# hazenai/SqueezeDet-PyTorch

Measured on AMD Instinct MI355X. Metric: images/sec SqueezeDet 1248x384 bs=20 inference (+ training under "train"), higher is better.
Workload: dtype f32; 1 GPU; SqueezeDet KITTI 1248x384 bs=20 inference on 1 MI355X (Fire+ConvDet HIP kernels, fused NMS); arch=squeezedet, global_batch=20, input=3x384x1248 fp32 NCHW, HBM resident, weights=synthetic Kaiming-scale, seed 1234, parallelism=replicas x1, steps_in_flight=2

## Files before the change

squeezedet-pytorch_amd/csrc/conv_wino.hip:

```cpp
#include "sqd_common.h"
#include "wino_tile.h"
#include <type_traits>

struct WinoArgs {
  const float* x; const float* u; const float* bias; float* y;
  int B, H, W;
  int C, x_pitch, x_coff;
  int N, Npad, y_pitch, y_coff;
  int relu, accumulate;
  const float* ymask; const float* ymul;
  int gxn, gyn;
  unsigned gxn_m, gyn_m;
  int ngroups, ntiles;
  int nslices, gx;
  int wg_cap;
  int nslices3, N1, y_coff1;
  const float* bias1;
  const float* br_w; const float* br_bias; const float* br_sqb;
  int br_nsq;
  int pb_hp, pb_wp, pb_ns, pb_nseg, pb_gseg, pb_ng;
  float* sv; int sv_pitch, sv_coff, sv_coff1;
  unsigned char* sv_codes;
};

typedef __attribute__((address_space(3))) void* lds_ptr_w_t;

template <int NT, int WV>
__global__ __launch_bounds__(WV * 64, (WV == 4 && NT == 2) ? 2 : ((WV == 4 && NT == 1) ? 3 : 1)) void conv_wino_kernel(WinoArgs a) {
#if defined(__HIP_DEVICE_COMPILE__)
  constexpr int NTHR = WV * 64;
  constexpr int BN = 16 * NT;
  constexpr int RAW_IT = 4;
  constexpr int USLOTS = 32 * BN;
  static_assert(USLOTS % NTHR == 0, "U slice must be whole workgroup passes");
  constexpr int U_IT = USLOTS / NTHR;
  constexpr int NDMA = RAW_IT + U_IT;
  constexpr int NSTEP = 8;
  extern __shared__ __attribute__((aligned(16))) float smem[];
  float* const rawB = smem;
  float* const VB = rawB + WV * 256 * 4;
  float* const UB = VB + WV * 1024 * NT;

  const int tid = threadIdx.x, lane = tid & 63, wv = tid >> 6;
  const int lr = lane & 15, g = lane >> 4;
  const int wgq = (int)blockIdx.x >> 3;
  const int n0 = (wgq % a.nslices) * BN;
  const int tstride = a.gx;
  const int nchunks = a.C >> 3;
  const int ntiles = a.ntiles;
  int tile = ((int)blockIdx.x & 7) * (a.gx >> 3) + wgq / a.nslices;
  if (tile >= ntiles) return;
  const int wv_s = __builtin_amdgcn_readfirstlane(wv);

  int r_offB[RAW_IT], r_key[RAW_IT];
#pragma unroll
  for (int it = 0; it < RAW_IT; ++it) wino_patch_slot(it * 64 + lane, a.W, a.x_pitch, r_offB[it], r_key[it]);
  int u_offB[U_IT];
#pragma unroll
  for (int it = 0; it < U_IT; ++it) {
    const int slot = it * NTHR + tid;
    const int pp = slot / (4 * BN), rem = slot - pp * (4 * BN);
    u_offB[it] = ((pp * a.Npad + n0) * 16 + rem * 4) * 4;
  }
  const unsigned u_chunkB = 16u * a.Npad * 8u * 4u;
  const __amdgpu_buffer_rsrc_t xres = __builtin_amdgcn_make_buffer_rsrc(
      (void*)(a.x + a.x_coff - (long long)(a.W + 1) * a.x_pitch), 0, 0x7ffffff0, 0x00020000);
  const __amdgpu_buffer_rsrc_t ures = __builtin_amdgcn_make_buffer_rsrc((void*)a.u, 0, 0x7ffffff0, 0x00020000);

  typedef WinoGPos GPos;
  auto group_pos = [&](int t) { return wino_group_pos(a, t * WV + wv_s); };
  int r_offG[RAW_IT];
  auto group_offsets = [&](const GPos gp) { wino_group_offsets<RAW_IT>(gp.y0, gp.x0, gp.inner, a.H, a.W, r_offB, r_key, r_offG); };
  float* const rawW = rawB + wv_s * 256 * 4;
  float* const VW = VB + wv_s * 1024 * NT;
  auto dma_raw_one = [&](int it, unsigned soff) {
    __builtin_amdgcn_raw_ptr_buffer_load_lds(xres, (lds_ptr_w_t)(rawW + it * 64 * 4), 16, r_offG[it], (int)soff, 0, 0);
  };
  auto dma_u_one = [&](int it, int cc, int buf) {
    __builtin_amdgcn_raw_ptr_buffer_load_lds(ures, (lds_ptr_w_t)(UB + (buf * USLOTS + it * NTHR + wv_s * 64) * 4), 16, u_offB[it],
                                             (int)(cc * u_chunkB), 0, 0);
  };

  f32x4 acc[16][NT];
#pragma unroll
  for (int p = 0; p < 16; ++p)
#pragma unroll
    for (int j = 0; j < NT; ++j) acc[p][j] = (f32x4){0.f, 0.f, 0.f, 0.f};

  f32x4 biasv[NT];
#pragma unroll
  for (int j = 0; j < NT; ++j) {
    const int n = n0 + j * 16 + 4 * g;
    biasv[j] = (a.bias && n < a.N) ? *(const f32x4*)(a.bias + n) : (f32x4){0.f, 0.f, 0.f, 0.f};
  }
  const int ty = lr >> 3, tx = lr & 7;
  int o_off[4];
#pragma unroll
  for (int px = 0; px < 4; ++px) o_off[px] = ((2 * ty + (px >> 1)) * a.W + 2 * tx + (px & 1)) * a.y_pitch + 4 * g;
  const float relu_lo = a.relu ? 0.f : -__builtin_inff();

  const float* const rawL = rawW + (((g >> 1) * WINO_RP + (2 * (lr >> 3)) * 18 + 2 * (lr & 7)) * 4 + 2 * (g & 1));
  const float* const uR0 = UB + g * 64 + lr * 4;
  f32x4* const parkW = (f32x4*)VW + lane;

  GPos cur = group_pos(tile);
  group_offsets(cur);
#pragma unroll
  for (int it = 0; it < RAW_IT; ++it) dma_raw_one(it, cur.soff);
#pragma unroll
  for (int it = 0; it < U_IT; ++it) dma_u_one(it, 0, 0);
  int ubuf = 0;
  bool pending = false;
  GPos ptp = cur;

  const int acc_i = a.accumulate, has_mul = a.ymul != nullptr, has_mask = a.ymask != nullptr;
  auto epi = [&](f32x4 v, int j, float* dst, const float* mul, const float* mask) {
    if (acc_i) v += *(const f32x4*)dst;
    if (has_mul) v *= *(const f32x4*)mul;
    if (has_mask) {
      const f32x4 m = *(const f32x4*)mask;
      v.x = m.x > 0.f ? v.x : 0.f; v.y = m.y > 0.f ? v.y : 0.f; v.z = m.z > 0.f ? v.z : 0.f; v.w = m.w > 0.f ? v.w : 0.f;
    }
    *(f32x4*)dst = wino_relu4(v, relu_lo);
  };
  auto flush = [&](const GPos gp) {
    float* ybase = a.y + gp.p0 * a.y_pitch + a.y_coff + n0;
    const float* mulbase = a.ymul + gp.p0 * a.y_pitch + a.y_coff + n0;
    const float* maskbase = a.ymask + gp.p0 * a.y_pitch + a.y_coff + n0;
    const bool whole = gp.y0 + 4 <= a.H && gp.x0 + 16 <= a.W && n0 + BN <= a.N;
    if (!gp.valid) return;
    if (whole) {
#pragma unroll
      for (int px = 0; px < 4; ++px)
#pragma unroll
        for (int j = 0; j < NT; ++j) {
          const int off = o_off[px] + j * 16;
          epi(parkW[(px * NT + j) * 64], j, ybase + off, mulbase + off, maskbase + off);
        }
      return;
    }
#pragma unroll
    for (int px = 0; px < 4; ++px) {
      const bool valid = gp.y0 + 2 * ty + (px >> 1) < a.H && gp.x0 + 2 * tx + (px & 1) < a.W;
#pragma unroll
      for (int j = 0; j < NT; ++j) {
        if (!valid || n0 + j * 16 + 4 * g >= a.N) continue;
        const int off = o_off[px] + j * 16;
        epi(parkW[(px * NT + j) * 64], j, ybase + off, mulbase + off, maskbase + off);
      }
    }
  };

  for (;;) {
    const int more_i = (int)((unsigned)(tile + tstride - ntiles) >> 31);
    const bool more = more_i != 0;
    const GPos nxt = group_pos(more ? tile + tstride : tile);
    for (int cc = 0; cc < nchunks; ++cc) {
      asm volatile("s_waitcnt vmcnt(0)" ::: "memory");
      __syncthreads();
      if (pending) { flush(ptp); pending = false; }
      const int last_i = 1 - (int)((unsigned)(cc + 1 - nchunks) >> 31);
      const bool last = last_i != 0;
      const int ncc = last ? 0 : cc + 1;
      if (last) group_offsets(nxt);
      const unsigned nsoff = (last ? nxt.soff : cur.soff) + (unsigned)ncc * 32u;

      f32x2 vv[16];
      wino_input_transform(rawL, vv);
      asm volatile("s_waitcnt lgkmcnt(0)" ::: "memory");
      __builtin_amdgcn_sched_barrier(0);
      const float* const uR = uR0 + ubuf * USLOTS * 4;

      auto load_ops = [&](int step, f32x4 (&afr)[NT]) {
#pragma unroll
        for (int j = 0; j < NT; ++j) afr[j] = *(const f32x4*)(uR + (step * NT + j) * 256);
      };
      auto mfma_phase = [&](auto first_c) {
      constexpr bool FIRST = decltype(first_c)::value;
      auto mfma_pos = [&](int step, const f32x4 (&afr)[NT], int h) {
        const int p = 2 * step + h;
#pragma unroll
        for (int t = 0; t < 2; ++t)
#pragma unroll
          for (int j = 0; j < NT; ++j) {
            const f32x4 c0v = (FIRST && t == 0) ? ((p == 5) ? biasv[j] : (f32x4){0.f, 0.f, 0.f, 0.f}) : acc[p][j];
            acc[p][j] = mfma16(afr[j][2 * h + t], vv[p][t], c0v);
          }
      };
      f32x4 af0[NT], af1[NT];
      load_ops(0, af0);
#pragma unroll
      for (int step = 0; step < NSTEP; ++step) {
#pragma unroll
        for (int q = 0; q < NDMA; ++q) {
          if (q * NSTEP / NDMA != step) continue;
          if (q < RAW_IT) dma_raw_one(q < RAW_IT ? q : 0, nsoff);
          else dma_u_one(q - RAW_IT, ncc, ubuf ^ 1);
        }
        if (step & 1) {
          mfma_pos(step, af1, 0);
          __builtin_amdgcn_sched_barrier(0);
          if (step + 1 < NSTEP) load_ops(step + 1, af0);
          __builtin_amdgcn_sched_barrier(0);
          mfma_pos(step, af1, 1);
        } else {
          mfma_pos(step, af0, 0);
          __builtin_amdgcn_sched_barrier(0);
          if (step + 1 < NSTEP) load_ops(step + 1, af1);
          __builtin_amdgcn_sched_barrier(0);
          mfma_pos(step, af0, 1);
        }
      }
      };
      if (cc == 0) mfma_phase(std::true_type{}); else mfma_phase(std::false_type{});

      if (last) {
#pragma unroll
        for (int j = 0; j < NT; ++j) {
          f32x4 ov[4];
          wino_inverse(acc, j, ov);
#pragma unroll
          for (int px = 0; px < 4; ++px) parkW[(px * NT + j) * 64] = ov[px];
        }
        pending = true; ptp = cur;
      }
      ubuf ^= 1;
    }
    if (!more) break;
    tile += tstride;
    cur = nxt;
  }
  if (pending) flush(ptp);
  asm volatile("s_waitcnt vmcnt(0)" ::: "memory");
#endif
}

template <int NT, int WV, bool USTAT, bool E1>
__device__ __forceinline__ void wino_pipe_body(const WinoArgs& a) {
  static_assert(USTAT, "streamed-U form retired");
  static_assert(!E1 || NT == 2, "expand1x1 slices are built on the 32-channel tiling");
  constexpr int NTHR = WV * 64;
  constexpr int BN = 16 * NT;
  constexpr int RAW_IT = 4;
  constexpr int USLOTS = 32 * BN;
  static_assert(USLOTS % NTHR == 0, "U slice must be whole workgroup passes");
  constexpr int U_IT = USLOTS / NTHR;
  constexpr int NDMA = RAW_IT;
  constexpr int NST = 4 * NT;
  constexpr int NSTEP = 8;
  constexpr int RAW_STEPS = 4;
  extern __shared__ __attribute__((aligned(16))) float smem[];
  float* const rawB = smem;
  float* const UB = rawB + 2 * WV * 256 * 4;

  const int tid = threadIdx.x, lane = tid & 63, wv = tid >> 6;
  const int lr = lane & 15, g = lane >> 4;
  const int wgq = (int)blockIdx.x >> 3;
  const int n0 = (wgq % a.nslices) * BN;
  const int tstride = a.gx;
  const int nchunks = a.C >> 3;
  const int ntiles = a.ntiles;
  int tile = ((int)blockIdx.x & 7) * (a.gx >> 3) + wgq / a.nslices;
  if (tile >= ntiles) return;
  const int wv_s = __builtin_amdgcn_readfirstlane(wv);

  int r_offB[RAW_IT], r_key[RAW_IT];
#pragma unroll
  for (int it = 0; it < RAW_IT; ++it) wino_patch_slot(it * 64 + lane, a.W, a.x_pitch, r_offB[it], r_key[it]);
  int u_offB[U_IT];
#pragma unroll
  for (int it = 0; it < U_IT; ++it) {
    const int slot = it * NTHR + tid;
    const int pp = slot / (4 * BN), rem = slot - pp * (4 * BN);
    u_offB[it] = ((pp * a.Npad + n0) * 16 + rem * 4) * 4;
  }
  const unsigned u_chunkB = 16u * a.Npad * 8u * 4u;
  const __amdgpu_buffer_rsrc_t xres = __builtin_amdgcn_make_buffer_rsrc(
      (void*)(a.x + a.x_coff - (long long)(a.W + 1) * a.x_pitch), 0, 0x7ffffff0, 0x00020000);
  const __amdgpu_buffer_rsrc_t ures = __builtin_amdgcn_make_buffer_rsrc((void*)a.u, 0, 0x7ffffff0, 0x00020000);

  typedef WinoGPos GPos;
  auto group_pos = [&](int t) { return wino_group_pos(a, t * WV + wv_s); };
  int r_offG[RAW_IT];
  auto group_offsets = [&](int y0, int x0, int inner) { wino_group_offsets<RAW_IT>(y0, x0, inner, a.H, a.W, r_offB, r_key, r_offG); };
  float* const rawW = rawB + wv_s * 256 * 4;
  auto dma_raw_one = [&](int it, unsigned soff, int rb) {
    __builtin_amdgcn_raw_ptr_buffer_load_lds(xres, (lds_ptr_w_t)(rawW + (rb * WV * 256 + it * 64) * 4), 16, r_offG[it], (int)soff, 0, 0);
  };
  auto dma_u_one = [&](int it, int cc, int slot) {
    __builtin_amdgcn_raw_ptr_buffer_load_lds(ures, (lds_ptr_w_t)(UB + (slot * USLOTS + it * NTHR + wv_s * 64) * 4), 16, u_offB[it],
                                             (int)(cc * u_chunkB), 0, 0);
  };

  f32x4 acc[16][NT];
#pragma unroll
  for (int p = 0; p < 16; ++p)
#pragma unroll
    for (int j = 0; j < NT; ++j) acc[p][j] = (f32x4){0.f, 0.f, 0.f, 0.f};
  f32x4 biasv[NT];
#pragma unroll
  for (int j = 0; j < NT; ++j) {
    const int n = n0 + j * 16 + 4 * g;
    biasv[j] = (!E1 && a.bias && n < a.N) ? *(const f32x4*)(a.bias + n) : (f32x4){0.f, 0.f, 0.f, 0.f};
  }
  const int e1_c0 = E1 ? (n0 - a.nslices3 * BN) * 4 : 0;
  float e1_biasA[E1 ? 8 : 1];
  const float e1_oneB = (g == 0) ? 1.f : 0.f;
  if constexpr (E1) {
#pragma unroll
    for (int blk = 0; blk < 8; ++blk) {
      const int ch = e1_c0 + blk * 16 + lr;
      e1_biasA[blk] = (g == 0 && a.bias1 && ch < a.N1) ? a.bias1[ch] : 0.f;
    }
  }
  const int ty = lr >> 3, tx = lr & 7;
  int o_offB[4];
#pragma unroll
  for (int px = 0; px < 4; ++px) o_offB[px] = (((2 * ty + (px >> 1)) * a.W + 2 * tx + (px & 1)) * a.y_pitch + 4 * g) * 4;
  const __amdgpu_buffer_rsrc_t yres = __builtin_amdgcn_make_buffer_rsrc((void*)(E1 ? a.y + a.y_coff1 + e1_c0 : a.y + a.y_coff + n0), 0, 0x7ffffff0, 0x00020000);
  const __amdgpu_buffer_rsrc_t mulres = __builtin_amdgcn_make_buffer_rsrc((void*)(a.ymul ? a.ymul + a.y_coff + n0 : a.y), 0, 0x7ffffff0, 0x00020000);
  const __amdgpu_buffer_rsrc_t maskres = __builtin_amdgcn_make_buffer_rsrc((void*)(a.ymask ? a.ymask + a.y_coff + n0 : a.y), 0, 0x7ffffff0, 0x00020000);
  const float relu_lo = a.relu ? 0.f : -__builtin_inff();
  const int rawL_off = (((g >> 1) * WINO_RP + (2 * (lr >> 3)) * 18 + 2 * (lr & 7)) * 4 + 2 * (g & 1));
// ... 500 lines not shown
```

squeezedet-pytorch_amd/csrc/wino_poolbridge.h:

```cpp
template <int NSQ, int NCH, bool SAVE = false>
__device__ __forceinline__ void wino_poolbridge16_body(const WinoArgs& a) {
  constexpr int WV = 8, NTHR = WV * 64, RAW_IT = 4, RSLOTS = 224;
  extern __shared__ __attribute__((aligned(16))) float smem[];
  const int P3 = a.nslices3, P = a.nslices;
  constexpr int nchunks = NCH;
  const bool e1_half = a.N1 <= 64;
  const int e1_stage = e1_half ? 1024 : 2048;
  const int rb1 = e1_half ? 2 : 4;
  float* const rawB = smem;
  float* const UB = rawB + 2 * WV * RSLOTS * 4;
  float* const U1B = UB + P3 * nchunks * 2048;
  float* const sqAL = U1B + (P - P3) * nchunks * e1_stage;
  const int nblk = P3 + rb1 * (P - P3);
  float* const biasL = sqAL + nblk * 4 * NSQ * 64;
  float* const sqbL = biasL + P * 64;

  const int tid = threadIdx.x, lane = tid & 63, wv = tid >> 6;
  const int lr = lane & 15, g = lane >> 4;
  const int ntasks = a.ngroups;
  const int wv_s = __builtin_amdgcn_readfirstlane(wv);
  int task = (int)blockIdx.x * WV + wv_s;
  const int tstride = a.gx * WV;

  int r_offB[RAW_IT], r_key[RAW_IT];
#pragma unroll
  for (int it = 0; it < RAW_IT; ++it) wino_patch_slot(it * 64 + lane, a.W, a.x_pitch, r_offB[it], r_key[it]);
  const __amdgpu_buffer_rsrc_t xres = __builtin_amdgcn_make_buffer_rsrc(
      (void*)(a.x + a.x_coff - (long long)(a.W + 1) * a.x_pitch), 0, 0x7ffffff0, 0x00020000);
  const __amdgpu_buffer_rsrc_t ures = __builtin_amdgcn_make_buffer_rsrc((void*)a.u, 0, 0x7ffffff0, 0x00020000);
  const __amdgpu_buffer_rsrc_t yres = __builtin_amdgcn_make_buffer_rsrc(
      (void*)(a.y + a.y_coff - (long long)a.pb_wp * a.y_pitch), 0, 0x7ffffff0, 0x00020000);
  const __amdgpu_buffer_rsrc_t pres = __builtin_amdgcn_make_buffer_rsrc(
      (void*)((SAVE ? a.sv : a.y) - (SAVE ? (long long)a.pb_wp * a.sv_pitch : 0)), 0, 0x7ffffff0, 0x00020000);
  const __amdgpu_buffer_rsrc_t cres = __builtin_amdgcn_make_buffer_rsrc(
      (void*)(SAVE ? (void*)(a.sv_codes - (long long)a.pb_wp * a.sv_pitch) : (void*)a.y), 0, 0x7ffffff0, 0x00020000);

  {
    const int u_lane = (g * 16 + lr) * 16;
    const unsigned u_chunkB = 16u * a.Npad * 8u * 4u;
    for (int ps = 0; ps < P; ++ps)
      for (int c = 0; c < nchunks; ++c) {
        const bool is1 = ps >= P3;
        if (is1 && e1_half && (wv_s & 1)) continue;
        float* const dst = is1 ? U1B + ((ps - P3) * nchunks + c) * e1_stage + (e1_half ? (wv_s >> 1) : wv_s) * 256
                               : UB + (ps * nchunks + c) * 2048 + wv_s * 256;
        __builtin_amdgcn_raw_ptr_buffer_load_lds(ures, (lds_ptr_w_t)dst, 16, u_lane + wv_s * a.Npad * 64,
                                                 (int)(c * u_chunkB + (unsigned)ps * 1024u), 0, 0);
      }
    for (int i = tid; i < nblk * 4 * NSQ * 64; i += NTHR) sqAL[i] = a.br_w[i];
    for (int i = tid; i < P * 64; i += NTHR) biasL[i] = a.br_bias[i];
    for (int i = tid; i < NSQ * 16; i += NTHR) sqbL[i] = (a.br_sqb && i < a.br_nsq) ? a.br_sqb[i] : 0.f;
  }
  asm volatile("s_waitcnt vmcnt(0)" ::: "memory");
  __syncthreads();
  if (task >= ntasks) return;

  struct IterPos { int b, s, r, y0, x0, inner; unsigned soff; };
  auto iter_pos = [&](int b, int s, int r) {
    IterPos ip;
    ip.b = b; ip.s = s; ip.r = r;
    ip.y0 = 4 * r; ip.x0 = 14 * s;
    const long long p0 = ((long long)b * a.H + ip.y0) * a.W + ip.x0;
    ip.soff = (unsigned)(p0 * a.x_pitch * 4);
    ip.inner = (int)(((unsigned)(-ip.y0) & (unsigned)(ip.y0 + 4 - a.H) & (unsigned)(-ip.x0) & (unsigned)(ip.x0 + 16 - a.W)) >> 31);
    return ip;
  };
  float* const rawW = rawB + wv_s * RSLOTS * 4;
  auto dma_group = [&](const IterPos& ip) {
#pragma unroll
    for (int it = 0; it < RAW_IT; ++it) {
      const int key = r_key[it];
      const bool ok = ip.inner ? true : (key >= 0 && (unsigned)(ip.y0 + (key >> 8) - 1) < (unsigned)a.H && (unsigned)(ip.x0 + (key & 255) - 1) < (unsigned)a.W);
      const int off = ok ? r_offB[it] : (int)WINO_OOB;
      if (it < RAW_IT - 1 || lane < RSLOTS - (RAW_IT - 1) * 64) {
        __builtin_amdgcn_raw_ptr_buffer_load_lds(xres, (lds_ptr_w_t)(rawW + (it * 64) * 4), 16, off, (int)ip.soff, 0, 0);
        if (nchunks > 1)
          __builtin_amdgcn_raw_ptr_buffer_load_lds(xres, (lds_ptr_w_t)(rawW + (WV * RSLOTS + it * 64) * 4), 16, off, (int)(ip.soff + 32u), 0, 0);
      }
    }
  };
  auto task_of = [&](int q, int& b, int& s, int& g0, int& g1) {
    const int v = q % a.pb_nseg; const int q1 = q / a.pb_nseg;
    s = q1 % a.pb_ns; b = q1 / a.pb_ns;
    g0 = v * a.pb_gseg; g1 = g0 + a.pb_gseg < a.pb_ng ? g0 + a.pb_gseg : a.pb_ng;
  };

  f32x4 acc[16];
  f32x4 acc_sq[NSQ];
  f32x4 carry[8];
  unsigned carry_code[SAVE ? 8 : 1];
#pragma unroll
  for (int k = 0; k < 8; ++k) carry[k] = (f32x4){0.f, 0.f, 0.f, 0.f};
#pragma unroll
  for (int k = 0; k < (SAVE ? 8 : 1); ++k) carry_code[k] = 0u;
  const float oneB = (g == 0) ? 1.f : 0.f;
  const int ty = lr >> 3, tx = lr & 7;
  const int o_off = (((1 - ty) * a.pb_wp + tx) * a.y_pitch + 4 * g) * 4;
  const int p_off = SAVE ? (((1 - ty) * a.pb_wp + tx) * a.sv_pitch + 4 * g) * 4 : 0;
  const int rawL_off = (((g >> 1) * WINO_RP + (2 * (lr >> 3)) * 18 + 2 * (lr & 7)) * 4 + 2 * (g & 1));
  const int u_ln = g * 64 + lr * 4;
  auto max4 = [](f32x4 p, f32x4 q) {
    f32x4 r;
    r.x = __builtin_fmaxf(p.x, q.x); r.y = __builtin_fmaxf(p.y, q.y); r.z = __builtin_fmaxf(p.z, q.z); r.w = __builtin_fmaxf(p.w, q.w);
    return r;
  };
  auto shl = [](float v, auto n_c) {
    constexpr int N = decltype(n_c)::value;
    return __builtin_bit_cast(float, __builtin_amdgcn_update_dpp(0, __builtin_bit_cast(int, v), 0x100 + N, 0xf, 0xf, true));
  };
  auto shr = [](float v, auto n_c) {
    constexpr int N = decltype(n_c)::value;
    return __builtin_bit_cast(float, __builtin_amdgcn_update_dpp(0, __builtin_bit_cast(int, v), 0x110 + N, 0xf, 0xf, true));
  };

  int tb, ts, g0, g1;
  task_of(task, tb, ts, g0, g1);
  int r = g0;
  IterPos cur = iter_pos(tb, ts, r);
  dma_group(cur);
  bool stored = false;

  for (;;) {
    const int rlast = (g1 < a.pb_ng || 2 * a.pb_ng - 1 < a.pb_hp) ? g1 : g1 - 1;
    int nb = tb, ns = ts, ng0 = g0, ng1 = g1, nr = r + 1, ntask = task;
    bool more = true;
    if (r >= rlast) {
      ntask = task + tstride;
      more = ntask < ntasks;
      if (more) { task_of(ntask, nb, ns, ng0, ng1); nr = ng0; } else { nr = r; }
    }
    if (stored && (!SAVE || nblk == 8)) asm volatile("s_waitcnt vmcnt(%0)" ::"n"(NSQ + (SAVE ? 16 : 0)) : "memory");
    else asm volatile("s_waitcnt vmcnt(0)" ::: "memory");
    asm volatile("" ::: "memory");
    f32x2 vv[NCH][16];
#pragma unroll
    for (int c = 0; c < NCH; ++c) wino_input_transform(rawW + c * WV * RSLOTS * 4 + rawL_off, vv[c]);
    asm volatile("s_waitcnt lgkmcnt(0)" ::: "memory");
    __builtin_amdgcn_sched_barrier(0);
    const IterPos nxt = iter_pos(nb, ns, nr);
    dma_group(nxt);

#pragma unroll
    for (int q = 0; q < NSQ; ++q) acc_sq[q] = (f32x4){0.f, 0.f, 0.f, 0.f};
    const bool wholexy = cur.y0 + 4 <= a.H && cur.x0 + 16 <= a.W;
    const bool emit_px = tx < 7 && 7 * ts + tx < a.pb_wp && 2 * r - ty < a.pb_hp && (ty ? (r > g0) : (r < g1));
    const unsigned psoff = SAVE ? (unsigned)((((long long)tb * a.pb_hp + 2 * r) * a.pb_wp + 7 * ts) * a.sv_pitch * 4) : 0u;
    auto pool_in = [&](int bi, auto kslot_c, f32x4 (&ov)[4], int cbase, int climit) {
      constexpr int KS = decltype(kslot_c)::value;
      if (!wholexy) {
#pragma unroll
        for (int px = 0; px < 4; ++px)
          if (!(cur.y0 + 2 * ty + (px >> 1) < a.H && cur.x0 + 2 * tx + (px & 1) < a.W)) ov[px] = (f32x4){0.f, 0.f, 0.f, 0.f};
      }
      const f32x4 m_top = max4(ov[0], ov[1]), m_left = max4(ov[0], ov[2]);
      const f32x4 m_all = max4(m_top, max4(ov[2], ov[3]));
      f32x4 A, Bt, pooled;
      const f32x4 ov0 = ov[0];
      asm volatile("s_nop 1\n\t"
                   "v_max_f32_dpp %0, %8, %12 row_shl:1 row_mask:0xf bank_mask:0xf bound_ctrl:1\n\t"
                   "v_max_f32_dpp %1, %9, %13 row_shl:1 row_mask:0xf bank_mask:0xf bound_ctrl:1\n\t"
                   "v_max_f32_dpp %2, %10, %14 row_shl:1 row_mask:0xf bank_mask:0xf bound_ctrl:1\n\t"
                   "v_max_f32_dpp %3, %11, %15 row_shl:1 row_mask:0xf bank_mask:0xf bound_ctrl:1\n\t"
                   "v_max_f32_dpp %4, %16, %20 row_shl:1 row_mask:0xf bank_mask:0xf bound_ctrl:1\n\t"
                   "v_max_f32_dpp %5, %17, %21 row_shl:1 row_mask:0xf bank_mask:0xf bound_ctrl:1\n\t"
                   "v_max_f32_dpp %6, %18, %22 row_shl:1 row_mask:0xf bank_mask:0xf bound_ctrl:1\n\t"
                   "v_max_f32_dpp %7, %19, %23 row_shl:1 row_mask:0xf bank_mask:0xf bound_ctrl:1"
                   : "=&v"(A.x), "=&v"(A.y), "=&v"(A.z), "=&v"(A.w), "=&v"(Bt.x), "=&v"(Bt.y), "=&v"(Bt.z), "=&v"(Bt.w)
                   : "v"(m_left.x), "v"(m_left.y), "v"(m_left.z), "v"(m_left.w), "v"(m_all.x), "v"(m_all.y), "v"(m_all.z), "v"(m_all.w),
                     "v"(ov0.x), "v"(ov0.y), "v"(ov0.z), "v"(ov0.w), "v"(m_top.x), "v"(m_top.y), "v"(m_top.z), "v"(m_top.w));
      f32x4 base;
#pragma unroll
      for (int e = 0; e < 4; ++e) base[e] = ty ? carry[KS][e] : A[e];
      asm volatile("s_nop 1\n\t"
                   "v_max_f32_dpp %0, %4, %8 row_shl:8 row_mask:0xf bank_mask:0xf bound_ctrl:1\n\t"
                   "v_max_f32_dpp %1, %5, %9 row_shl:8 row_mask:0xf bank_mask:0xf bound_ctrl:1\n\t"
                   "v_max_f32_dpp %2, %6, %10 row_shl:8 row_mask:0xf bank_mask:0xf bound_ctrl:1\n\t"
                   "v_max_f32_dpp %3, %7, %11 row_shl:8 row_mask:0xf bank_mask:0xf bound_ctrl:1\n\t"
                   "v_max_f32_dpp %0, %4, %0 row_shr:8 row_mask:0xf bank_mask:0xf bound_ctrl:1\n\t"
                   "v_max_f32_dpp %1, %5, %1 row_shr:8 row_mask:0xf bank_mask:0xf bound_ctrl:1\n\t"
                   "v_max_f32_dpp %2, %6, %2 row_shr:8 row_mask:0xf bank_mask:0xf bound_ctrl:1\n\t"
                   "v_max_f32_dpp %3, %7, %3 row_shr:8 row_mask:0xf bank_mask:0xf bound_ctrl:1"
                   : "=&v"(pooled.x), "=&v"(pooled.y), "=&v"(pooled.z), "=&v"(pooled.w)
                   : "v"(Bt.x), "v"(Bt.y), "v"(Bt.z), "v"(Bt.w), "v"(base.x), "v"(base.y), "v"(base.z), "v"(base.w));
      if constexpr (SAVE) {
        unsigned codes = 0u, cApack = 0u;
#pragma unroll
        for (int e = 0; e < 4; ++e) {
          const float o0 = ov[0][e], o1 = ov[1][e], o2 = ov[2][e], o3 = ov[3][e];
          float r0;
          asm volatile("s_nop 1\n\tv_mov_b32_dpp %0, %1 row_shl:1 row_mask:0xf bank_mask:0xf bound_ctrl:1" : "=&v"(r0) : "v"(o0));
          const float Av = A[e], Bv = Bt[e];
          unsigned cA = 5u;
          cA = (o3 == Av) ? 4u : cA; cA = (o2 == Av) ? 3u : cA; cA = (r0 == Av) ? 2u : cA; cA = (o1 == Av) ? 1u : cA; cA = (o0 == Av) ? 0u : cA;
          const unsigned cB = (o0 == Bv) ? 6u : ((o1 == Bv) ? 7u : 8u);
          unsigned cBn;
          asm volatile("s_nop 1\n\t"
                       "v_mov_b32_dpp %0, %1 row_shl:8 row_mask:0xf bank_mask:0x3 bound_ctrl:1\n\t"
                       "v_mov_b32_dpp %0, %1 row_shr:8 row_mask:0xf bank_mask:0xc bound_ctrl:1" : "=&v"(cBn) : "v"(cB));
          const unsigned cbase_e = ty ? ((carry_code[KS] >> (8 * e)) & 0xffu) : cA;
          unsigned code = (base[e] == pooled[e]) ? cbase_e : cBn;
          code = pooled[e] > 0.f ? code : 15u;
          codes |= code << (8 * e);
          cApack |= cA << (8 * e);
          __builtin_amdgcn_sched_barrier(0);
        }
        carry_code[KS] = cApack;
        pooled = wino_relu4(pooled, 0.f);
        const bool st = emit_px && cbase + 4 * g < climit;
        const int pv = st ? p_off + cbase * 4 : (int)WINO_OOB;
        wino_store16(pooled, pres, pv, (int)psoff);
        __builtin_amdgcn_raw_buffer_store_b32(codes, cres, st ? (p_off >> 2) + cbase : (int)WINO_OOB, (int)(psoff >> 2), 0);
        __builtin_amdgcn_sched_barrier(0);
        asm volatile("s_nop 1" ::: "memory");
        __builtin_amdgcn_sched_barrier(0);
      } else {
        pooled = wino_relu4(pooled, 0.f);
      }
      carry[KS] = A;
      const float* const sA = sqAL + bi * (4 * NSQ * 64) + lane;
#pragma unroll
      for (int t = 0; t < 4; ++t)
#pragma unroll
        for (int q = 0; q < NSQ; ++q) acc_sq[q] = mfma16(sA[(t * NSQ + q) * 64], pooled[t], acc_sq[q]);
    };

    {
      auto run_pass = [&](auto kind_c, auto kslot_c, int pass) {
        constexpr int KIND = decltype(kind_c)::value;
        constexpr int KS0 = decltype(kslot_c)::value;
        constexpr bool E1 = KIND != 0;
        constexpr int SSTEP = (KIND == 2) ? 2 : 1, NS = 8 / SSTEP;
        const float* const bL = biasL + pass * 64 + lr;
        float bA[E1 ? 4 : 1];
#pragma unroll
        for (int k = 0; k < (E1 ? (KIND == 2 ? 2 : 4) : 1); ++k) bA[k] = bL[k * 16];
        {
          auto chunk = [&](auto first_c, auto cc_c) {
            constexpr int cc = decltype(cc_c)::value;
            const float* const uR = (E1 ? U1B + ((pass - P3) * nchunks + cc) * e1_stage : UB + (pass * nchunks + cc) * 2048) + u_ln;
            constexpr bool FIRST = decltype(first_c)::value;
            constexpr int CC = decltype(cc_c)::value;
            f32x4 af0 = *(const f32x4*)uR, af1;
#pragma unroll
            for (int si = 0; si < NS; ++si) {
              const int step = si * SSTEP;
              __builtin_amdgcn_sched_barrier(0);
              if (si + 1 < NS) { if (si & 1) af0 = *(const f32x4*)(uR + (si + 1) * 256); else af1 = *(const f32x4*)(uR + (si + 1) * 256); }
              __builtin_amdgcn_sched_barrier(0);
              const f32x4 af = (si & 1) ? af1 : af0;
#pragma unroll
              for (int t = 0; t < 2; ++t)
#pragma unroll
                for (int h = 0; h < 2; ++h) {
                  const int p = 2 * step + h;
                  const int pv = E1 ? ((p >> 2) == 0 ? 5 : (p >> 2) == 1 ? 6 : (p >> 2) == 2 ? 9 : 10) : p;
                  f32x4 c0v;
                  if (FIRST && t == 0) {
                    c0v = (f32x4){0.f, 0.f, 0.f, 0.f};
                    if (E1 ? (p < 4) : (p == 5)) c0v = mfma16(bA[E1 ? (p & 3) : 0], oneB, c0v);
                  } else {
                    c0v = acc[p];
                  }
                  acc[p] = mfma16(af[2 * h + t], vv[CC][pv][t], c0v);
                }
            }
          };
          chunk(std::true_type{}, std::integral_constant<int, 0>{});
          if constexpr (NCH > 1) chunk(std::false_type{}, std::integral_constant<int, 1>{});
        }
        if constexpr (E1) {
          const int bi0 = P3 + rb1 * (pass - P3);
#pragma unroll
          for (int rr = 0; rr < (KIND == 2 ? 2 : 4); ++rr) {
            f32x4 ov[4];
            wino_inverse_inner(acc, rr, ov);
            const int s1 = pass - P3, c1 = a.sv_coff1 + 128 * (s1 >> 1) + (2 * rr + (s1 & 1)) * 16, l1 = a.sv_coff1 + a.N1;
            if (rr == 0) pool_in(bi0 + rr, std::integral_constant<int, KS0>{}, ov, c1, l1);
            else if (rr == 1) pool_in(bi0 + rr, std::integral_constant<int, KS0 + 1>{}, ov, c1, l1);
            else if (rr == 2) pool_in(bi0 + rr, std::integral_constant<int, (KS0 + 2) & 7>{}, ov, c1, l1);
            else pool_in(bi0 + rr, std::integral_constant<int, (KS0 + 3) & 7>{}, ov, c1, l1);
          }
        } else {
          f32x4 ov[4];
          wino_inverse(acc, ov);
          pool_in(pass, std::integral_constant<int, KS0>{}, ov, a.sv_coff + 16 * pass, a.sv_coff + a.N);
        }
      };
      if (P3 > 0) run_pass(std::integral_constant<int, 0>{}, std::integral_constant<int, 0>{}, 0);
      if (P3 > 1) run_pass(std::integral_constant<int, 0>{}, std::integral_constant<int, 1>{}, 1);
      if (P3 > 2) run_pass(std::integral_constant<int, 0>{}, std::integral_constant<int, 2>{}, 2);
      if (P3 > 3) run_pass(std::integral_constant<int, 0>{}, std::integral_constant<int, 3>{}, 3);
      if (e1_half) {
        if (P > P3) run_pass(std::integral_constant<int, 2>{}, std::integral_constant<int, 4>{}, P3);
        if (P > P3 + 1) run_pass(std::integral_constant<int, 2>{}, std::integral_constant<int, 6>{}, P3 + 1);
      }
    }
    {
      const int prow = 2 * r - ty, pcol = 7 * ts + tx;
      const bool emit = tx < 7 && pcol < a.pb_wp && prow < a.pb_hp && (ty ? (r > g0) : (r < g1));
      const unsigned ysoff = (unsigned)((((long long)tb * a.pb_hp + 2 * r) * a.pb_wp + 7 * ts) * a.y_pitch * 4);
#pragma unroll
      for (int q = 0; q < NSQ; ++q) {
        const f32x4 v = wino_relu4(acc_sq[q] + *(const f32x4*)(sqbL + q * 16 + 4 * g), 0.f);
        const int voff = (emit && q * 16 + 4 * g < a.br_nsq) ? o_off + q * 64 : (int)WINO_OOB;
        wino_store16(v, yres, voff, (int)ysoff);
      }
      stored = true;
    }
    if (!more) break;
    task = ntask; tb = nb; ts = ns; g0 = ng0; g1 = ng1; r = nr;
    cur = nxt;
  }
  asm volatile("s_waitcnt vmcnt(0)" ::: "memory");
}

template <int NSQ, int NCH, bool SAVE>
__global__ __launch_bounds__(512, 1) void fire_poolbridge16_kernel(WinoArgs a) {
#if defined(__HIP_DEVICE_COMPILE__)
  wino_poolbridge16_body<NSQ, NCH, SAVE>(a);
#endif
}

template <int NSQ, int NCH, bool SAVE>
static int launch_wino_poolbridge16_t(WinoArgs a, int nseg, hipStream_t stream) {
  constexpr int WV = 8, NTHR = WV * 64, RSLOTS = 224;
  const int nchunks = a.C >> 3;
  if (nchunks != NCH) return SQD_ERR_UNSUPPORTED;
  const int P1 = 2 * sqd_cdiv(a.N1, 128);
  if (a.Npad != sqd_cdiv(a.N, 32) * 32 + sqd_cdiv(a.N1, 128) * 32) return SQD_ERR_BAD_ARG;
  const int first1 = sqd_cdiv(a.N, 32) * 2;
  const int e1_stage = a.N1 <= 64 ? 1024 : 2048, rb1 = a.N1 <= 64 ? 2 : 4;
  if (first1 > 4 || a.N1 > 64 || P1 > 2) return SQD_ERR_UNSUPPORTED;
  const int nblk = first1 + rb1 * P1;
  const size_t lds = (size_t)(2 * WV * RSLOTS * 4 + first1 * nchunks * 2048 + P1 * nchunks * e1_stage + nblk * 4 * NSQ * 64 + (first1 + P1) * 64 + NSQ * 16) * sizeof(float);
  if (lds > 160 * 1024) return SQD_ERR_UNSUPPORTED;
  if (SAVE && (!a.sv || !a.sv_codes)) return SQD_ERR_BAD_ARG;
  auto kern = fire_poolbridge16_kernel<NSQ, NCH, SAVE>;
  static SqdDevOnce attr_once;
  if (int rc_attr = sqd_max_lds_once(attr_once, (const void*)kern, 160 * 1024)) return rc_attr;
  a.pb_ng = sqd_cdiv(a.H, 4);
  a.pb_ns = sqd_cdiv(a.pb_wp, 7);
  if (nseg < 1) nseg = 1;
  if (nseg > a.pb_ng) nseg = a.pb_ng;
  a.pb_gseg = sqd_cdiv(a.pb_ng, nseg);
  a.pb_nseg = sqd_cdiv(a.pb_ng, a.pb_gseg);
  a.ngroups = a.B * a.pb_ns * a.pb_nseg;
  const int gx = sqd_even_grid(sqd_cdiv(a.ngroups, WV), sqd_num_cus());
  a.nslices3 = first1; a.nslices = first1 + P1; a.gx = gx;
  hipLaunchKernelGGL(kern, dim3((unsigned)gx), dim3(NTHR), lds, stream, a);
  return sqd_launch_status();
}

template <int NSQ, bool SAVE = false>
static int launch_wino_poolbridge16(WinoArgs a, int nseg, hipStream_t stream) {
  if ((a.C >> 3) == 1) return launch_wino_poolbridge16_t<NSQ, 1, SAVE>(a, nseg, stream);
  if ((a.C >> 3) == 2) return launch_wino_poolbridge16_t<NSQ, 2, SAVE>(a, nseg, stream);
  return SQD_ERR_UNSUPPORTED;
}
```

Before: 15170 images/sec.

## Share seam rows between adjacent row-segment waves via LDS instead of recomputing

When the pool-bridge kernel splits rows into segments, each segment previously computed one extra Winograd group at its lower boundary to produce the pooled seam row. In the new seam mode, each wave parks its first-group pooled partials in registers and writes them to LDS at the end of its segment. After a workgroup barrier, the neighbouring wave in the ring reads them and finishes the seam row with its own carry. This removes the redundant extra-group convolution and input DMA per segment, at the cost of workgroup barriers that couple the waves, extra register pressure, and the restriction that nseg divides 8. Segment boundaries are also rebalanced to an even split.

```diff
diff --git a/squeezedet-pytorch_amd/csrc/conv_wino.hip b/squeezedet-pytorch_amd/csrc/conv_wino.hip
--- a/squeezedet-pytorch_amd/csrc/conv_wino.hip
+++ b/squeezedet-pytorch_amd/csrc/conv_wino.hip
@@ -18,7 +18,7 @@
   const float* bias1;
   const float* br_w; const float* br_bias; const float* br_sqb;
   int br_nsq;
-  int pb_hp, pb_wp, pb_ns, pb_nseg, pb_gseg, pb_ng;
+  int pb_hp, pb_wp, pb_ns, pb_nseg, pb_seam, pb_ng;
   float* sv; int sv_pitch, sv_coff, sv_coff1;
   unsigned char* sv_codes;
 };
diff --git a/squeezedet-pytorch_amd/csrc/wino_poolbridge.h b/squeezedet-pytorch_amd/csrc/wino_poolbridge.h
--- a/squeezedet-pytorch_amd/csrc/wino_poolbridge.h
+++ b/squeezedet-pytorch_amd/csrc/wino_poolbridge.h
@@ -1,5 +1,6 @@
-template <int NSQ, int NCH, bool SAVE = false>
+template <int NSQ, int NCH, bool SAVE = false, bool SEAM = false>
 __device__ __forceinline__ void wino_poolbridge16_body(const WinoArgs& a) {
+  static_assert(!(SAVE && SEAM), "the storing form keeps the extra-group path");
   constexpr int WV = 8, NTHR = WV * 64, RAW_IT = 4, RSLOTS = 224;
   extern __shared__ __attribute__((aligned(16))) float smem[];
   const int P3 = a.nslices3, P = a.nslices;
@@ -53,7 +54,10 @@
   }
   asm volatile("s_waitcnt vmcnt(0)" ::: "memory");
   __syncthreads();
-  if (task >= ntasks) return;
+  if (task >= ntasks) {
+    if (SEAM && task - wv_s < ntasks) __builtin_amdgcn_s_barrier();
+    return;
+  }
 
   struct IterPos { int b, s, r, y0, x0, inner; unsigned soff; };
   auto iter_pos = [&](int b, int s, int r) {
@@ -65,7 +69,9 @@
     ip.inner = (int)(((unsigned)(-ip.y0) & (unsigned)(ip.y0 + 4 - a.H) & (unsigned)(-ip.x0) & (unsigned)(ip.x0 + 16 - a.W)) >> 31);
     return ip;
   };
-  float* const rawW = rawB + wv_s * RSLOTS * 4;
+  int ring = wv_s;
+  const int ring_end = SEAM ? (wv_s & ~(a.pb_nseg - 1)) + a.pb_nseg : 0;
+  float* rawW = rawB + ring * RSLOTS * 4;
   auto dma_group = [&](const IterPos& ip) {
 #pragma unroll
     for (int it = 0; it < RAW_IT; ++it) {
@@ -82,13 +88,16 @@
   auto task_of = [&](int q, int& b, int& s, int& g0, int& g1) {
     const int v = q % a.pb_nseg; const int q1 = q / a.pb_nseg;
     s = q1 % a.pb_ns; b = q1 / a.pb_ns;
-    g0 = v * a.pb_gseg; g1 = g0 + a.pb_gseg < a.pb_ng ? g0 + a.pb_gseg : a.pb_ng;
+    g0 = v * a.pb_ng / a.pb_nseg; g1 = (v + 1) * a.pb_ng / a.pb_nseg;
   };
 
   f32x4 acc[16];
   f32x4 acc_sq[NSQ];
   f32x4 carry[8];
   unsigned carry_code[SAVE ? 8 : 1];
+  f32x4 park[SEAM ? 4 : 1];
+#pragma unroll
+  for (int k = 0; k < (SEAM ? 4 : 1); ++k) park[k] = (f32x4){0.f, 0.f, 0.f, 0.f};
 #pragma unroll
   for (int k = 0; k < 8; ++k) carry[k] = (f32x4){0.f, 0.f, 0.f, 0.f};
 #pragma unroll
@@ -121,10 +130,12 @@
   bool stored = false;
 
   for (;;) {
-    const int rlast = (g1 < a.pb_ng || 2 * a.pb_ng - 1 < a.pb_hp) ? g1 : g1 - 1;
+    const int rlast = SEAM ? g1 - 1 : ((g1 < a.pb_ng || 2 * a.pb_ng - 1 < a.pb_hp) ? g1 : g1 - 1);
     int nb = tb, ns = ts, ng0 = g0, ng1 = g1, nr = r + 1, ntask = task;
     bool more = true;
-    if (r >= rlast) {
+    const bool last = r >= rlast;
+    const bool park_it = SEAM && r == g0 && g0 > 0;
+    if (last) {
       ntask = task + tstride;
       more = ntask < ntasks;
       if (more) { task_of(ntask, nb, ns, ng0, ng1); nr = ng0; } else { nr = r; }
@@ -138,7 +149,7 @@
     asm volatile("s_waitcnt lgkmcnt(0)" ::: "memory");
     __builtin_amdgcn_sched_barrier(0);
     const IterPos nxt = iter_pos(nb, ns, nr);
-    dma_group(nxt);
+    if (!(SEAM && last)) dma_group(nxt);
 
 #pragma unroll
     for (int q = 0; q < NSQ; ++q) acc_sq[q] = (f32x4){0.f, 0.f, 0.f, 0.f};
@@ -168,6 +179,20 @@
                    : "=&v"(A.x), "=&v"(A.y), "=&v"(A.z), "=&v"(A.w), "=&v"(Bt.x), "=&v"(Bt.y), "=&v"(Bt.z), "=&v"(Bt.w)
                    : "v"(m_left.x), "v"(m_left.y), "v"(m_left.z), "v"(m_left.w), "v"(m_all.x), "v"(m_all.y), "v"(m_all.z), "v"(m_all.w),
                      "v"(ov0.x), "v"(ov0.y), "v"(ov0.z), "v"(ov0.w), "v"(m_top.x), "v"(m_top.y), "v"(m_top.z), "v"(m_top.w));
+      if constexpr (SEAM) {
+        if (park_it) {
+          if constexpr ((KS & 1) == 0) {
+            park[KS >> 1] = Bt;
+          } else {
+#pragma unroll
+            for (int e = 0; e < 4; ++e) {
+              const float keep = park[KS >> 1][e], top = Bt[e];
+              park[KS >> 1][e] = __builtin_bit_cast(float, __builtin_amdgcn_update_dpp(__builtin_bit_cast(int, keep), __builtin_bit_cast(int, top),
+                                                                                      0x118, 0xf, 0xc, false));
+            }
+          }
+        }
+      }
       f32x4 base;
 #pragma unroll
       for (int e = 0; e < 4; ++e) base[e] = ty ? carry[KS][e] : A[e];
@@ -307,17 +332,77 @@
       }
       stored = true;
     }
+    if constexpr (SEAM) {
+      if (last) {
+        if (g0 > 0) {
+#pragma unroll
+          for (int j = 0; j < 4; ++j) *(f32x4*)(rawW + (j >> 1) * (WV * RSLOTS * 4) + ((j & 1) * 64 + lane) * 4) = park[j];
+        }
+        asm volatile("s_waitcnt lgkmcnt(0)\n\ts_barrier" ::: "memory");
+        ring = ring + 1 == ring_end ? ring_end - a.pb_nseg : ring + 1;
+        rawW = rawB + ring * RSLOTS * 4;
+        const bool below = g1 < a.pb_ng;
+        if (below || 2 * a.pb_ng - 1 < a.pb_hp) {
+          f32x4 in[4];
+#pragma unroll
+          for (int j = 0; j < 4; ++j) in[j] = (f32x4){0.f, 0.f, 0.f, 0.f};
+          if (below) {
+#pragma unroll
+            for (int j = 0; j < 4; ++j) in[j] = *(const f32x4*)(rawW + (j >> 1) * (WV * RSLOTS * 4) + ((j & 1) * 64 + lane) * 4);
+          }
+#pragma unroll
+          for (int q = 0; q < NSQ; ++q) acc_sq[q] = (f32x4){0.f, 0.f, 0.f, 0.f};
+          auto finish = [&](auto kslot_c, int bi) {
+            constexpr int KS = decltype(kslot_c)::value;
+            f32x4 bt = in[KS >> 1], pooled;
+            if constexpr ((KS & 1) == 0) {
+#pragma unroll
+              for (int e = 0; e < 4; ++e) bt[e] = shr(bt[e], std::integral_constant<int, 8>{});
+            }
+#pragma unroll
+            for (int e = 0; e < 4; ++e) pooled[e] = __builtin_fmaxf(bt[e], __builtin_fmaxf(0.f, carry[KS][e]));
+            pooled = wino_relu4(pooled, 0.f);
+            const float* const sA = sqAL + bi * (4 * NSQ * 64) + lane;
+#pragma unroll
+            for (int t = 0; t < 4; ++t)
+#pragma unroll
+              for (int q = 0; q < NSQ; ++q) acc_sq[q] = mfma16(sA[(t * NSQ + q) * 64], pooled[t], acc_sq[q]);
+          };
+          if (P3 > 0) finish(std::integral_constant<int, 0>{}, 0);
+          if (P3 > 1) finish(std::integral_constant<int, 1>{}, 1);
+          if (P3 > 2) finish(std::integral_constant<int, 2>{}, 2);
+          if (P3 > 3) finish(std::integral_constant<int, 3>{}, 3);
+          if (P > P3) { finish(std::integral_constant<int, 4>{}, P3); finish(std::integral_constant<int, 5>{}, P3 + 1); }
+          if (P > P3 + 1) { finish(std::integral_constant<int, 6>{}, P3 + 2); finish(std::integral_constant<int, 7>{}, P3 + 3); }
+          const bool emit = ty && tx < 7 && 7 * ts + tx < a.pb_wp && 2 * g1 - 1 < a.pb_hp;
+          const unsigned ysoff = (unsigned)((((long long)tb * a.pb_hp + 2 * g1) * a.pb_wp + 7 * ts) * a.y_pitch * 4);
+#pragma unroll
+          for (int q = 0; q < NSQ; ++q) {
+            const f32x4 v = wino_relu4(acc_sq[q] + *(const f32x4*)(sqbL + q * 16 + 4 * g), 0.f);
+            const int voff = (emit && q * 16 + 4 * g < a.br_nsq) ? o_off + q * 64 : (int)WINO_OOB;
+            wino_store16(v, yres, voff, (int)ysoff);
+          }
+        }
+        asm volatile("s_waitcnt lgkmcnt(0)" ::: "memory");
+        if (more) dma_group(nxt);
+        stored = false;
+      }
+    }
     if (!more) break;
     task = ntask; tb = nb; ts = ns; g0 = ng0; g1 = ng1; r = nr;
     cur = nxt;
   }
   asm volatile("s_waitcnt vmcnt(0)" ::: "memory");
+  if (SEAM && task + tstride - wv_s < ntasks) __builtin_amdgcn_s_barrier();
 }
 
 template <int NSQ, int NCH, bool SAVE>
 __global__ __launch_bounds__(512, 1) void fire_poolbridge16_kernel(WinoArgs a) {
 #if defined(__HIP_DEVICE_COMPILE__)
-  wino_poolbridge16_body<NSQ, NCH, SAVE>(a);
+  if constexpr (!SAVE) {
+    if (a.pb_seam) { wino_poolbridge16_body<NSQ, NCH, false, true>(a); return; }
+  }
+  wino_poolbridge16_body<NSQ, NCH, SAVE, false>(a);
 #endif
 }
 
@@ -342,8 +427,8 @@
   a.pb_ns = sqd_cdiv(a.pb_wp, 7);
   if (nseg < 1) nseg = 1;
   if (nseg > a.pb_ng) nseg = a.pb_ng;
-  a.pb_gseg = sqd_cdiv(a.pb_ng, nseg);
-  a.pb_nseg = sqd_cdiv(a.pb_ng, a.pb_gseg);
+  a.pb_nseg = nseg;
+  a.pb_seam = !SAVE && 8 % nseg == 0;
   a.ngroups = a.B * a.pb_ns * a.pb_nseg;
   const int gx = sqd_even_grid(sqd_cdiv(a.ngroups, WV), sqd_num_cus());
   a.nslices3 = first1; a.nslices = first1 + P1; a.gx = gx;
```

Result: no change. 15250 images/sec (median of 3 runs) (+0.5%).
